# CX9898/BSMR-SDDMM

Hardware: AMD Instinct MI355X
Metric: SDDMM GFLOP/s (higher is better)
Workload: dtype f16

## Files before the change

### bsmr-sddmm_amd/csrc/bsmr_capi.hip

```cpp

#include "bsmr_hip.h"

#include <hip/hip_runtime.h>
#include <hipcub/hipcub.hpp>

#include <algorithm>
#include <chrono>
#include <cmath>
#include <cstdio>
#include <cstdlib>
#include <cstring>
#include <initializer_list>
#include <map>
#include <memory>
#include <mutex>
#include <new>
#include <set>
#include <string>
#include <type_traits>
#include <vector>

#include "dev_array.hpp"
#include "cluster_kernels.hpp"
#include "pack_device.hpp"
// ... 37 lines not shown
    uint32_t H = 0;
    DevArray<uint32_t> groupRows;
    DevArray<uint32_t> blockCols;
    DevArray<uint32_t> blockInfo;
    DevArray<uint32_t> entries;
    DevArray<bsmr::TileItem> items;
    DevArray<uint32_t> itemRowBase;
    uint32_t numItems = 0, entryCap = 0, blocksPerItem = 0;
    uint64_t numBlocks = 0, numTiles = 0, unionColumns = 0, bytes = 0;
};

struct SweepFormatDev {
    uint32_t W = 0, PW = 0, stripBlocks = 0;
    DevArray<uint32_t> panelRows;
    DevArray<bsmr::SweepItem> items;
    DevArray<uint32_t> starts;
    DevArray<uint32_t> rowStart;
    DevArray<uint32_t> words;
    uint32_t numItems = 0, numGroups = 0, numStrips = 0, maxStepEntries = 0, maxItemWords = 0;
    uint64_t bytes = 0;
    bool usable = false;
};

struct GemmFormatDev {
    uint32_t PM = 0, NB = 0;
    DevArray<uint32_t> panelRows;
    DevArray<uint32_t> colOf;
    DevArray<bsmr::GemmItem> items;
    DevArray<uint32_t> rowStart;
    DevArray<uint32_t> lists;
    DevArray<uint32_t> words;
    uint32_t numItems = 0, numGroups = 0, numStrips = 0;
    uint64_t numTiles = 0, bytes = 0;
    bool fullGrid = false, usable = false;
};

struct bsmr_plan {
    int device = 0;
    uint32_t M = 0, N = 0, nnz = 0, numPanels = 0;

    DenseFormat fmt[2];
    uint64_t numDenseEntries = 0;

    DevArray<uint32_t> panelRows;
    DevArray<uint32_t> entryCol;
    DevArray<uint32_t> entryDst;
    DevArray<uint8_t> entryRow;
    DevArray<SparseItem> sparseItems;
    uint64_t numSparseEntries = 0;
    uint32_t numSparseItems = 0;

    uint64_t indexBytes = 0;

    DevArray<uint16_t> A16;
    DevArray<uint16_t> B16;
    uint32_t reservedK = 0;

    int sparseLpe = 0;
    bool sparseLowp = true;
    bool convertInKernel = false;
    DevArray<uint32_t> entryRowId;
    bool sparseFree = false;
    uint64_t foldedEntries = 0;
    uint64_t promotedEntries = 0;
    uint64_t evictedEntries = 0;
    bool groupedDeferred = false;
    bsmr::PackOptions groupedOpt;
// ... 1179 lines not shown
    std::stable_sort(order.begin(), order.end());
    const uint32_t pick = order[std::min<size_t>((size_t)rank, order.size() - 1)].second;
    PM = kGemmShapes[pick][0];
    NB = kGemmShapes[pick][1];
}

int ensureGemm(bsmr_plan* p, uint32_t K) {
    uint32_t PM, NB;
    gemmShape(p, K, PM, NB);
    p->gemmNow = -1;
    if (!gemmShapeBuilt(PM, NB, gemmFp32(p, K))) return BSMR_OK;
    for (size_t i = 0; i < p->gemms.size(); ++i)
        if (p->gemms[i].PM == PM && p->gemms[i].NB == NB) {
            if (p->gemms[i].usable) p->gemmNow = (int)i;
            return BSMR_OK;
        }
    try {
        GemmFormatDev w;
        w.PM = PM;
        w.NB = NB;
        bsmr::GemmFormatHost host;
        int st = bsmr::packGemm(p->hostDense, PM, NB, host, p->opt.gemm_balance_columns != 0);
        if (st == BSMR_ERR_BAD_PLAN || st == BSMR_ERR_INVALID_ARG) {
            p->gemms.push_back(std::move(w));
            return BSMR_OK;
        }
        if (st != BSMR_OK) return st;
        uint64_t bytes = 0;
        w.numItems = (uint32_t)host.items.size();
        w.numGroups = host.numGroups;
        w.numStrips = host.numStrips;
        w.numTiles = host.numTiles;
        w.fullGrid = host.fullGrid;
        st = upload(w.panelRows, host.panelRows, bytes);
        if (st == BSMR_OK) st = upload(w.colOf, host.colOf, bytes);
        if (st == BSMR_OK) st = upload(w.items, host.items, bytes);
        if (st == BSMR_OK) st = upload(w.rowStart, host.rowStart, bytes);
        if (st == BSMR_OK) st = upload(w.lists, host.lists, bytes);
        if (st == BSMR_OK) st = upload(w.words, host.words, bytes);
        if (st != BSMR_OK) return st;
        w.bytes = bytes;
        w.usable = w.numItems != 0;
        p->gemms.push_back(std::move(w));
        p->indexBytes += bytes;
        if (p->gemms.back().usable) p->gemmNow = (int)p->gemms.size() - 1;
        return BSMR_OK;
    } catch (const std::bad_alloc&) {
        return BSMR_ERR_OOM;
    }
}

template <int KT, int PM, int NB, int MODE, bool SRC32>
int launchGemmT(const GemmFormatDev& w, const bsmr_plan* p, const void* A, const void* B, float* P, const Queue& s) {
    const uint64_t K = (SRC32 ? 32u : 64u) * KT, esz = SRC32 ? 4 : 2;
    const uint32_t aBytes = (uint32_t)((uint64_t)p->M * K * esz), bBytes = (uint32_t)((uint64_t)p->N * K * esz);
    const dim3 grid(w.numItems, s.batch.count), block(bsmr::kGemmWaves * bsmr::kWave);
    if constexpr (SRC32) {
        auto kernel = bsmr::denseGemmCvt<KT, PM, NB, MODE>;
        const size_t lds = bsmr::gemmCvtLdsBytes(PM, NB);
        if (int st = raiseDynamicLds(reinterpret_cast<const void*>(kernel), lds, p->device)) return st;
        hipLaunchKernelGGL(kernel, grid, block, lds, s, static_cast<const float*>(A), static_cast<const float*>(B), aBytes, bBytes, w.panelRows,
                           w.colOf, w.items, w.rowStart, w.lists, w.words, P, p->N, w.numGroups, w.numStrips, w.fullGrid ? 1u : 0u, s.batch);
    } else {
        auto kernel = bsmr::denseGemm<KT, PM, NB, MODE, false>;
        const size_t lds = bsmr::gemmLdsBytes(PM, NB);
        if (int st = raiseDynamicLds(reinterpret_cast<const void*>(kernel), lds, p->device)) return st;
        hipLaunchKernelGGL(kernel, grid, block, lds, s, A, B, aBytes, bBytes, w.panelRows, w.colOf, w.items, w.rowStart, w.lists, w.words, P, p->N,
                           w.numGroups, w.numStrips, w.fullGrid ? 1u : 0u, s.batch);
    }
    BSMR_HIP(hipGetLastError());
    return BSMR_OK;
}
template <int KT, int MODE, bool SRC32>
int launchGemmS(const GemmFormatDev& w, const bsmr_plan* p, const void* A, const void* B, float* P, const Queue& s) {
    switch (w.PM * 100 + w.NB) {
    case 1616: return launchGemmT<KT, 16, 16, MODE, SRC32>(w, p, A, B, P, s);
    case 1620: return launchGemmT<KT, 16, 20, MODE, SRC32>(w, p, A, B, P, s);
    case 816: return launchGemmT<KT, 8, 16, MODE, SRC32>(w, p, A, B, P, s);
    case 820: return launchGemmT<KT, 8, 20, MODE, SRC32>(w, p, A, B, P, s);
    case 1612:
        if constexpr (!SRC32) return launchGemmT<KT, 16, 12, MODE, false>(w, p, A, B, P, s);
        return BSMR_ERR_INVALID_ARG;
    default: return BSMR_ERR_INVALID_ARG;
    }
}
template <int MODE>
int launchGemm(const bsmr_plan* p, uint32_t K, const void* A, const void* B, float* P, const Queue& s, bool src32) {
    const GemmFormatDev& w = p->gemms[(size_t)p->gemmNow];
    if (w.numItems == 0) return BSMR_OK;
    if (src32) {
        switch (K) {
        case 64: return launchGemmS<2, MODE, true>(w, p, A, B, P, s);
        case 128: return launchGemmS<4, MODE, true>(w, p, A, B, P, s);
        default: return BSMR_ERR_INVALID_ARG;
        }
    }
    switch (K) {
    case 64: return launchGemmS<1, MODE, false>(w, p, A, B, P, s);
    case 128: return launchGemmS<2, MODE, false>(w, p, A, B, P, s);
    case 256: return launchGemmS<4, MODE, false>(w, p, A, B, P, s);
    case 512: return launchGemmS<8, MODE, false>(w, p, A, B, P, s);
// ... 1945 lines not shown
```

### bsmr-sddmm_amd/csrc/gemm_format.hpp

```cpp
#pragma once

#include <algorithm>
#include <cstdint>
#include <vector>

#include "bsmr_hip.h"
#include "tile_format.hpp"

namespace bsmr {

constexpr uint32_t kGemmWavesM = 2, kGemmWavesN = 4, kGemmWaves = kGemmWavesM * kGemmWavesN;
__host__ __device__ constexpr uint32_t gemmSlabSlot(uint32_t tp, uint32_t r, uint32_t c) { return tp * 256u + (r & 3u) * 64u + (r >> 2) * 16u + c; }
constexpr uint32_t kGemmPassTiles = 16;
constexpr uint32_t kGemmNoEntry = 0xFFFFFFFFu;
constexpr uint32_t kGemmMaxOffset = 8191u;
constexpr uint32_t kGemmSlabStrips = 8;
constexpr uint32_t kGemmWordSlack = 1024;
constexpr uint32_t kGemmMaxRowTiles = 8, kGemmMaxPasses = 3;

struct GemmItem {
    uint32_t group;
    uint32_t firstBlock;
    uint32_t listBase;
    uint32_t pad;
};

__host__ __device__ inline void gemmItemPlace(uint32_t i, uint32_t G, uint32_t S, uint32_t& group, uint32_t& strip) {
    const uint32_t slabs = (S + kGemmSlabStrips - 1u) / kGemmSlabStrips;
    uint32_t slab = i / (kGemmSlabStrips * G);
    if (slab >= slabs) slab = slabs - 1u;
    const uint32_t width = slab + 1u < slabs ? kGemmSlabStrips : S - kGemmSlabStrips * (slabs - 1u);
    const uint32_t rem = i - slab * kGemmSlabStrips * G;
    group = rem / width;
    strip = slab * kGemmSlabStrips + rem % width;
}

struct GemmFormatHost {
    uint32_t PM = 0, NB = 0, numGroups = 0, numStrips = 0, passes = 0;
    bool fullGrid = false;
    std::vector<uint32_t> panelRows;
    std::vector<uint32_t> colOf;
    std::vector<GemmItem> items;
    std::vector<uint32_t> rowStart;
    std::vector<uint32_t> lists;
    std::vector<uint32_t> words;
    uint64_t numTiles = 0;
    uint32_t maxListWords = 0;
    size_t bytes() const {
        return 4 * (panelRows.size() + colOf.size() + rowStart.size() + lists.size() + words.size()) + sizeof(GemmItem) * items.size();
    }
};

inline bool gemmShapeOk(uint32_t PM, uint32_t NB) {
    return (PM == 8 || PM == 16) && (NB == 8 || NB == 12 || NB == 16 || NB == 20);
}

inline int packGemm(const HostDense& hd, uint32_t PM, uint32_t NB, GemmFormatHost& out, bool balanceColumns = true) {
    if (!gemmShapeOk(PM, NB)) return BSMR_ERR_INVALID_ARG;
    const uint32_t P = hd.numPanels, TM = PM * 16;
    const uint32_t G = (P + PM - 1) / PM, NCB = (hd.N + 15) / 16, S = (NCB + NB - 1) / NB;
    const uint32_t m = PM / kGemmWavesM, n = NB / kGemmWavesN, Q = (m * n + kGemmPassTiles - 1) / kGemmPassTiles, L = kGemmWaves * Q;
    out = GemmFormatHost();
    out.PM = PM; out.NB = NB; out.numGroups = G; out.numStrips = S; out.passes = Q;
    if (P == 0 || NCB == 0 || hd.entries() == 0) return BSMR_OK;
    if ((uint64_t)G * S > 0x3FFFFFFFull || hd.entries() > 0xFFFFFFF0ull) return BSMR_ERR_INVALID_ARG;
    if ((uint64_t)hd.nnz * 4u > 0xFFFFFFFCull) return BSMR_ERR_INVALID_ARG;
    out.panelRows.assign((size_t)G * TM, hd.panelRows.empty() ? 0u : hd.panelRows[0]);
    std::vector<uint32_t> rowPos((size_t)P * 16);
    if (balanceColumns) {
        std::vector<uint32_t> weight((size_t)P * 16, 0), order((size_t)P * 16);
        for (uint32_t p = 0; p < P; ++p)
            for (uint64_t e = hd.offsets[p]; e < hd.offsets[p + 1]; ++e) ++weight[(size_t)p * 16 + hd.row[e]];
        for (uint32_t i = 0; i < P * 16; ++i) order[i] = i;
        std::stable_sort(order.begin(), order.end(), [&](uint32_t a, uint32_t b) { return weight[a] > weight[b]; });
        const uint32_t bins = 2 * G, half = TM / 2;
        uint32_t share[kGemmMaxRowTiles][kGemmMaxPasses] = {};
        for (uint32_t tm = 0; tm < m; ++tm)
            for (uint32_t tn = 0; tn < n; ++tn) ++share[tm][(tm * n + tn) / kGemmPassTiles];
        std::vector<uint64_t> load((size_t)bins * Q, 0);
        std::vector<uint8_t> rowsIn((size_t)bins * m, 0);
        for (uint32_t rank = 0; rank < P * 16; ++rank) {
            const uint32_t round = rank / bins, pos = rank % bins, bin = (round & 1u) ? bins - 1u - pos : pos;
            const uint64_t w = weight[order[rank]];
            uint64_t* ld = &load[(size_t)bin * Q];
// ... 14 lines not shown
    for (uint32_t i = 0; i < P * 16; ++i) out.panelRows[rowPos[i]] = hd.panelRows[i];
    const uint32_t TN = NB * 16;
    std::vector<uint32_t> slotOf(hd.N);
    out.colOf.assign((size_t)S * TN, 0u);
    if (balanceColumns) {
        std::vector<uint32_t> degree(hd.N, 0), hot;
        for (uint64_t e = 0; e < hd.entries(); ++e) ++degree[hd.col[e]];
        uint64_t fullest = 0;
        for (uint32_t st = 0; st < S; ++st) {
            uint64_t sum = 0;
            for (uint32_t c = st * TN; c < std::min<uint64_t>(hd.N, (uint64_t)(st + 1) * TN); ++c) sum += degree[c];
            fullest = std::max(fullest, sum);
        }
        const bool lopsided = fullest * S > 2ull * hd.entries();
        const uint64_t threshold = lopsided ? 2ull * hd.entries() / std::max<uint32_t>(1u, hd.N) + 1ull : ~0ull;
        for (uint32_t c = 0; c < hd.N; ++c)
            if (degree[c] > threshold) hot.push_back(c);
        std::stable_sort(hot.begin(), hot.end(), [&](uint32_t a, uint32_t b) { return degree[a] > degree[b]; });
        std::vector<uint32_t> filled(S, 0);
        for (uint32_t rank = 0; rank < hot.size(); ++rank) {
            const uint32_t round = rank / S, pos = rank % S, strip = (round & 1u) ? S - 1u - pos : pos;
            slotOf[hot[rank]] = strip * TN + filled[strip]++;
        }
        uint32_t strip = 0;
        for (uint32_t c = 0; c < hd.N; ++c) {
            if (degree[c] > threshold) continue;
            while (filled[strip] == TN) ++strip;
            slotOf[c] = strip * TN + filled[strip]++;
        }
    } else {
        for (uint32_t c = 0; c < hd.N; ++c) slotOf[c] = c;
    }
    for (uint32_t c = 0; c < hd.N; ++c) out.colOf[slotOf[c]] = c;
    std::vector<uint32_t> itemOf((size_t)G * S, 0xFFFFFFFFu);
    std::vector<uint8_t> used((size_t)G * S, 0);
    for (uint32_t p = 0; p < P; ++p)
        for (uint64_t e = hd.offsets[p]; e < hd.offsets[p + 1]; ++e)
            used[(size_t)(rowPos[(size_t)p * 16 + hd.row[e]] / TM) * S + slotOf[hd.col[e]] / TN] = 1;
    for (uint32_t i = 0; i < G * S; ++i) {
        uint32_t g, st;
        gemmItemPlace(i, G, S, g, st);
        if (!used[(size_t)g * S + st]) continue;
        itemOf[(size_t)g * S + st] = (uint32_t)out.items.size();
        GemmItem it;
        it.group = g;
        it.firstBlock = st * NB;
        it.listBase = (uint32_t)(out.items.size() * (L + 1));
        it.pad = 0;
        out.items.push_back(it);
    }
    out.fullGrid = out.items.size() == (size_t)G * S;
    const size_t I = out.items.size();
    out.numTiles = (uint64_t)I * PM * NB;
    if (I * (size_t)(L + 1) > 0xFFFFFFFFull || I * (size_t)TM > 0xFFFFFFFFull) return BSMR_ERR_INVALID_ARG;
    out.lists.assign(I * (L + 1), 0);
    out.rowStart.assign(I * TM, 0xFFFFFFFFu);
    auto locate = [&](uint32_t p, uint64_t e, size_t& item, uint32_t& list, uint32_t& slot, uint32_t& rowInWave, uint32_t& rowInTile) {
        const uint32_t place = rowPos[(size_t)p * 16 + hd.row[e]];
        const uint32_t g = place / TM, pj = (place % TM) / 16u;
        const uint32_t slotCol = slotOf[hd.col[e]];
        const uint32_t cb = slotCol >> 4, s = cb / NB, bj = cb % NB;
        const uint32_t wm = pj / m, tm = pj % m, wn = bj / n, tn = bj % n;
        const uint32_t t = tm * n + tn, q = t / kGemmPassTiles, tp = t % kGemmPassTiles;
        const uint32_t r = place & 15u, c = slotCol & 15u;
        item = itemOf[(size_t)g * S + s];
        list = (wm * kGemmWavesN + wn) * Q + q;
// ... 58 lines not shown
```

### bsmr-sddmm_amd/csrc/gemm_kernels.hpp

```cpp
#pragma once

#include <hip/hip_runtime.h>
#include <stdint.h>

#include "gemm_format.hpp"
#include "sddmm_kernels.hpp"

namespace bsmr {

constexpr uint32_t kGemmBK = 64;
constexpr uint32_t kGemmRowBytes = kGemmBK * 2u;
__host__ __device__ constexpr uint32_t gemmSwz16(uint32_t row) { return (row >> 1) & 7u; }
__host__ __device__ constexpr uint32_t gemmSwz32(uint32_t row) { return ((row >> 1) & 1u) | (((row >> 3) & 1u) * 6u); }
constexpr uint32_t gemmStageBytes(int PM, int NB) { return (uint32_t)(PM + NB) * 16u * kGemmRowBytes; }
constexpr uint32_t kGemmSlabBytes = kGemmPassTiles * 1024u;
constexpr uint32_t gemmRingBytes(int PM, int NB) {
    return 2u * gemmStageBytes(PM, NB) > kGemmWaves * kGemmSlabBytes ? 2u * gemmStageBytes(PM, NB) : kGemmWaves * kGemmSlabBytes;
}
constexpr size_t gemmLdsBytes(int PM, int NB) { return gemmRingBytes(PM, NB) + (size_t)PM * 16u * 4u; }

#if defined(BSMR_GEMM_LAB)
#define GEMM_LAB_ARG , uint32_t labSkip, unsigned long long* labStamps
#define GEMM_LAB_SKIP(bit) (labSkip & (1u << (bit)))
#define GEMM_LAB_STAMPS unsigned long long labStamp[8] = {0, 0, 0, 0, 0, 0, 0, 0}
// ... 5 lines not shown
#define GEMM_LAB_ARG
#define GEMM_LAB_SKIP(bit) false
#define GEMM_LAB_STAMPS
#define GEMM_LAB_STAMP(i)
#define GEMM_LAB_STAMPS_OUT
#endif

__device__ __forceinline__ void gemmKeep(const u32x4& x) {
#if defined(__HIP_DEVICE_COMPILE__)
    asm volatile("" ::"v"(x));
#else
    (void)x;
#endif
}

constexpr uint32_t kGemmDumpHigh = 64764u;
__device__ __forceinline__ void gemmDumpTile(const f32x4& a, uint32_t tileAddr, bool high) {
#if defined(__HIP_DEVICE_COMPILE__)
#pragma clang diagnostic push
#pragma clang diagnostic ignored "-Winline-asm"
    if (!high)
        asm volatile("s_mov_b32 m0, %4\n\ts_nop 0\n\tds_write_addtid_b32 %0\n\tds_write_addtid_b32 %1 offset:256\n\t"
                     "ds_write_addtid_b32 %2 offset:512\n\tds_write_addtid_b32 %3 offset:768"
                     ::"v"(a[0]), "v"(a[1]), "v"(a[2]), "v"(a[3]), "s"(tileAddr) : "memory", "m0");
    else
        asm volatile("s_mov_b32 m0, %4\n\ts_nop 0\n\tds_write_addtid_b32 %0 offset:64764\n\tds_write_addtid_b32 %1 offset:65020\n\t"
                     "ds_write_addtid_b32 %2 offset:65276\n\tds_write_addtid_b32 %3 offset:65532"
                     ::"v"(a[0]), "v"(a[1]), "v"(a[2]), "v"(a[3]), "s"(tileAddr - kGemmDumpHigh) : "memory", "m0");
#pragma clang diagnostic pop
#else
    (void)a; (void)tileAddr; (void)high;
#endif
}
__device__ __forceinline__ uint32_t gemmLdsAddress(const void* p) {
    return (uint32_t)(uintptr_t)(__attribute__((address_space(3))) const void*)p;
}

template <uint32_t DMAS>
__device__ __forceinline__ void gemmStagePart(const uint8_t* src, uint32_t srcBytes, uint8_t* dst, uint32_t wave, const uint32_t* voff, uint32_t kOff) {
    const auto rsrc = __builtin_amdgcn_make_buffer_rsrc(const_cast<uint8_t*>(src), 0, srcBytes, 0x00020000);
#pragma unroll
    for (uint32_t j = 0; j < DMAS; ++j)
        __builtin_amdgcn_raw_ptr_buffer_load_lds(rsrc, (__attribute__((address_space(3))) void*)(dst + (wave * DMAS + j) * 1024u), 16, voff[j], kOff, 0, 0);
}
__device__ __forceinline__ void gemmStoreEntry(float* P, bool live, uint32_t index, float val) {
    const auto rsrc = __builtin_amdgcn_make_buffer_rsrc(P, 0, 0xFFFFFFFC, 0x00020000);
    __builtin_amdgcn_raw_buffer_store_b32(__builtin_bit_cast(uint32_t, val), rsrc, live ? index << 2 : 0xFFFFFFFFu, 0, 0);
}
template <uint32_t C>
__device__ __forceinline__ void gemmLoadWords(const uint32_t* __restrict__ words, uint32_t e0, uint32_t lane, uint32_t (&w)[C], bool skip) {
    const uint32_t* __restrict__ base = words + e0;
#pragma unroll
    for (uint32_t u = 0; u < C; ++u) w[u] = skip ? kGemmNoEntry : base[u * kWave + lane];
}
template <uint32_t C, uint32_t HALF>
__device__ __forceinline__ void gemmMaskTrip(const float* slab, const uint32_t* rowTable, float* P, uint32_t e, uint32_t last, uint32_t lane,
                                             const uint32_t (&w)[C], bool skipStores) {
#pragma unroll
    for (uint32_t u = 0; u < C; ++u) {
        const bool live = e + u * kWave + lane < last && w[u] != kGemmNoEntry;
        const float val = slab[w[u] & 4095u];
        const uint32_t dst = rowTable[(w[u] >> 12) & (HALF - 1u)] + (w[u] >> 19);
        if (!skipStores) gemmStoreEntry(P, live, dst, val);
    }
}
template <uint32_t C, uint32_t HALF, uint32_t Q, bool DEEP>
__device__ __forceinline__ void gemmMaskPass(const uint32_t* __restrict__ words, const float* slab, const uint32_t* rowTable, float* P,
                                             const uint32_t (&myList)[Q + 1u], uint32_t q, uint32_t lane, uint32_t (&wAhead)[2][C],
                                             bool skipLoads, bool skipStores) {
    const uint32_t first = myList[q], last = myList[q + 1u];
    uint32_t w[C];
#pragma unroll
    for (uint32_t u = 0; u < C; ++u) w[u] = wAhead[q & 1u][u];
    if (DEEP) {
        if (q + 2u < Q) gemmLoadWords<C>(words, myList[q + 2u], lane, wAhead[q & 1u], skipLoads);
    } else if (q + 1u < Q) {
        gemmLoadWords<C>(words, last, lane, wAhead[(q + 1u) & 1u], skipLoads);
    }
    constexpr uint32_t T = C * kWave;
    const bool more = first + T < last;
    uint32_t over[C];
    if (more) gemmLoadWords<C>(words, first + T, lane, over, skipLoads);
    gemmMaskTrip<C, HALF>(slab, rowTable, P, first, last, lane, w, skipStores);
    if (more) {
        for (uint32_t e = first + T; e < last; e += T) {
            uint32_t ahead[C];
            gemmLoadWords<C>(words, e + T, lane, ahead, skipLoads);
            gemmMaskTrip<C, HALF>(slab, rowTable, P, e, last, lane, over, skipStores);
#pragma unroll
            for (uint32_t u = 0; u < C; ++u) over[u] = ahead[u];
        }
    }
}
template <uint32_t ADMAS, uint32_t BDMAS>
__device__ __forceinline__ void gemmStage(const uint8_t* A, uint32_t aBytes, const uint8_t* B, uint32_t bBytes, uint8_t* stage, uint32_t bAt,
                                          uint32_t wave, const uint32_t* voffA, const uint32_t* voffB, uint32_t kOff) {
    gemmStagePart<BDMAS>(B, bBytes, stage + bAt, wave, voffB, kOff);
    gemmStagePart<ADMAS>(A, aBytes, stage, wave, voffA, kOff);
}
__device__ __forceinline__ uint32_t gemmRowOfLane(const uint32_t* __restrict__ rows8, uint32_t sub) {
    uint32_t id = rows8[0];
#pragma unroll
    for (uint32_t k = 1; k < 8; ++k) id = sub == k ? rows8[k] : id;
    return id;
}

template <int KT, int PM, int NB, int MODE, bool SRC32 = false>
__global__ void __launch_bounds__(kGemmWaves * kWave, 2)
denseGemm(const void* __restrict__ Aop, const void* __restrict__ Bop, uint32_t aBytes, uint32_t bBytes,
          const uint32_t* __restrict__ panelRows, const uint32_t* __restrict__ colOf, const GemmItem* __restrict__ items,
          const uint32_t* __restrict__ rowStart,
          const uint32_t* __restrict__ lists, const uint32_t* __restrict__ words, float* __restrict__ P, uint32_t N,
          uint32_t gridG, uint32_t gridS, uint32_t fullGrid, Batch batch GEMM_LAB_ARG) {
    constexpr uint32_t ESZ = SRC32 ? 4u : 2u, K = (kGemmRowBytes / ESZ) * KT, TM = PM * 16u, TN = NB * 16u;
    constexpr uint32_t KSUB = SRC32 ? 1u : 2u;
    constexpr uint32_t m = PM / kGemmWavesM, n = NB / kGemmWavesN, Q = (m * n + kGemmPassTiles - 1u) / kGemmPassTiles, L = kGemmWaves * Q;
    constexpr uint32_t ADMAS = PM / 4u, BDMAS = NB / 4u;
    static_assert(PM % 4 == 0 && NB % 4 == 0, "a stage is filled in whole 1-KiB pieces per wave");
    constexpr uint32_t stageBytes = gemmStageBytes(PM, NB), bAt = TM * kGemmRowBytes;
    constexpr uint32_t rowTableAt = gemmRingBytes(PM, NB);
    constexpr uint32_t kGemmWordChunk = m * n > 32u ? 4u : 8u;
    constexpr bool kPlainDump = m * n > 32u;

    extern __shared__ __attribute__((aligned(16))) uint8_t lds[];
    const uint32_t itemId = xcdContiguous(blockIdx.x, gridDim.x);
    uint32_t group, firstBlock, listBase;
    if (fullGrid) {
        gemmItemPlace(itemId, gridG, gridS, group, firstBlock);
        firstBlock *= (uint32_t)NB;
        listBase = itemId * (L + 1u);
    } else {
        const GemmItem item = items[itemId];
        group = item.group;
        firstBlock = item.firstBlock;
        listBase = item.listBase;
    }
    const uint32_t wave = __builtin_amdgcn_readfirstlane(threadIdx.x >> 6), lane = threadIdx.x & 63u;
    const uint32_t wm = wave / kGemmWavesN, wn = wave % kGemmWavesN;
    const uint32_t r = lane & 15u, g = lane >> 4;
    GEMM_LAB_STAMPS;
    GEMM_LAB_STAMP(0);

    const uint8_t* Ab = static_cast<const uint8_t*>(Aop) + (size_t)blockIdx.y * batch.strideA * ESZ;
    const uint8_t* Bb = static_cast<const uint8_t*>(Bop) + (size_t)blockIdx.y * batch.strideB * ESZ;
    P += (size_t)blockIdx.y * batch.strideP;

    uint32_t voffA[ADMAS], voffB[BDMAS];
#pragma unroll
    for (uint32_t j = 0; j < BDMAS; ++j) {
        const uint32_t col = 8u * (wave * BDMAS + j) + (lane >> 3);
        const uint32_t id = gemmRowOfLane(colOf + (size_t)firstBlock * 16u + 8u * (wave * BDMAS + j), lane >> 3);
        voffB[j] = id * (K * ESZ) + (((lane & 7u) ^ (SRC32 ? gemmSwz32(col) : gemmSwz16(col))) << 4);
    }
    if (!GEMM_LAB_SKIP(2)) gemmStagePart<BDMAS>(Bb, bBytes, lds + bAt, wave, voffB, 0u);
#pragma unroll
    for (uint32_t j = 0; j < ADMAS; ++j) {
        const uint32_t row = 8u * (wave * ADMAS + j) + (lane >> 3);
        const uint32_t id = gemmRowOfLane(panelRows + (size_t)group * TM + 8u * (wave * ADMAS + j), lane >> 3);
        voffA[j] = id * (K * ESZ) + (((lane & 7u) ^ (SRC32 ? gemmSwz32(row) : gemmSwz16(row))) << 4);
    }
    if (!GEMM_LAB_SKIP(2)) gemmStagePart<ADMAS>(Ab, aBytes, lds, wave, voffA, 0u);
    GEMM_LAB_STAMP(1);
    if (threadIdx.x < TM) reinterpret_cast<uint32_t*>(lds + rowTableAt)[threadIdx.x] = rowStart[(size_t)itemId * TM + threadIdx.x];
    uint32_t myList[Q + 1];
#pragma unroll
    for (uint32_t q = 0; q <= Q; ++q) myList[q] = lists[listBase + wave * Q + q];

    const uint32_t fragOff = r * kGemmRowBytes + ((SRC32 ? (2u * g) ^ gemmSwz32(r) : g ^ gemmSwz16(r)) << 4);
    const uint32_t aRead = wm * (TM / 2u) * kGemmRowBytes + fragOff;
    const uint32_t bRead = bAt + wn * (TN / 4u) * kGemmRowBytes + fragOff;

    f32x4 acc[m][n];
#pragma unroll
    for (uint32_t i = 0; i < m; ++i)
#pragma unroll
        for (uint32_t j = 0; j < n; ++j) acc[i][j] = f32x4{0.f, 0.f, 0.f, 0.f};

    auto loadWords = [&](uint32_t e0, uint32_t (&w)[kGemmWordChunk]) { gemmLoadWords<kGemmWordChunk>(words, e0, lane, w, GEMM_LAB_SKIP(4)); };
    constexpr bool kDeepWords = Q >= 2u && m * n <= 32u;
    uint32_t wAhead[2][kGemmWordChunk];
    constexpr bool kEarlyWords = KT <= 4 && !kPlainDump;
    auto firstWords = [&]() {
        loadWords(myList[0], wAhead[0]);
        if (kDeepWords) loadWords(myList[1], wAhead[1]);
    };
#if !defined(BSMR_GEMM_LATE_WORDS)
    if (kEarlyWords) firstWords();
#endif

    asm volatile("s_waitcnt vmcnt(0)" ::: "memory");
    GEMM_LAB_STAMP(2);
    __builtin_amdgcn_s_barrier();
    GEMM_LAB_STAMP(3);
#if defined(BSMR_GEMM_LATE_WORDS)
    if (kEarlyWords) firstWords();
#endif

#pragma unroll
    for (uint32_t t = 0; t < (uint32_t)KT; ++t) {
        if (t + 1u < (uint32_t)KT && !GEMM_LAB_SKIP(2))
            gemmStage<ADMAS, BDMAS>(Ab, aBytes, Bb, bBytes, lds + ((t + 1u) & 1u) * stageBytes, bAt, wave, voffA, voffB, (t + 1u) * kGemmRowBytes);
        if (!kEarlyWords && t + 1u == (uint32_t)KT) firstWords();
        const uint8_t* base = lds + (t & 1u) * stageBytes;
#pragma unroll
        for (uint32_t s = 0; s < KSUB; ++s) {
            auto fragment = [&](uint32_t at, uint32_t tile, uint32_t tag) -> u32x4 {
                if (GEMM_LAB_SKIP(1)) return u32x4{lane, t, tile, s + tag};
                const uint8_t* src = base + ((at + tile * 16u * kGemmRowBytes) ^ (s << 6));
                if constexpr (SRC32) {
                    const f32x4 lo = *reinterpret_cast<const f32x4*>(src);
                    const f32x4 hi = *reinterpret_cast<const f32x4*>(reinterpret_cast<const uint8_t*>(reinterpret_cast<uintptr_t>(src) ^ 16u));
                    return packLowp<MODE>(lo, hi);
                } else {
                    return *reinterpret_cast<const u32x4*>(src);
                }
            };
            u32x4 bf[n];
#pragma unroll
            for (uint32_t j = 0; j < n; ++j) bf[j] = fragment(bRead, j, 0u);
#pragma unroll
            for (uint32_t i = 0; i < m; ++i) {
                const u32x4 af = fragment(aRead, i, 2u);
                if (!GEMM_LAB_SKIP(0)) {
// ... 31 lines not shown
                for (uint32_t tp = 0; tp < kGemmPassTiles; ++tp) {
                    const uint32_t tIdx = q * kGemmPassTiles + tp;
                    if (tIdx < m * n) gemmDumpTile(acc[tIdx / n][tIdx % n], slabAddr + tp * 1024u, false);
                }
            } else {
#pragma unroll
                for (uint32_t tp = 0; tp < kGemmPassTiles; ++tp) {
                    const uint32_t tIdx = q * kGemmPassTiles + tp;
                    if (tIdx < m * n) gemmDumpTile(acc[tIdx / n][tIdx % n], slabAddr + tp * 1024u, true);
                }
            }
        }
        if (kPlainDump) __builtin_amdgcn_sched_barrier(0);
        gemmMaskPass<kGemmWordChunk, TM / 2u, Q, kDeepWords>(words, slab, rowTable, P, myList, q, lane, wAhead, GEMM_LAB_SKIP(4), GEMM_LAB_SKIP(5));
        GEMM_LAB_STAMP(5u + q);
    }
    GEMM_LAB_STAMPS_OUT;
}

constexpr uint32_t kGemmHalfRowBytes = 64u;
__host__ __device__ constexpr uint32_t gemmSwzH(uint32_t row) { return (4u - ((row >> 2) & 3u)) & 3u; }
constexpr uint32_t gemmCvtRingBytes(int PM, int NB) {
    const uint32_t used = (uint32_t)(PM + NB) * 16u * (kGemmRowBytes + 2u * kGemmHalfRowBytes);
    return used > kGemmWaves * kGemmSlabBytes ? used : kGemmWaves * kGemmSlabBytes;
}
constexpr size_t gemmCvtLdsBytes(int PM, int NB) { return gemmCvtRingBytes(PM, NB) + (size_t)PM * 16u * 4u; }

template <int KT, int PM, int NB, int MODE>
__global__ void __launch_bounds__(kGemmWaves * kWave, 2)
denseGemmCvt(const float* __restrict__ Aop, const float* __restrict__ Bop, uint32_t aBytes, uint32_t bBytes,
             const uint32_t* __restrict__ panelRows, const uint32_t* __restrict__ colOf, const GemmItem* __restrict__ items,
             const uint32_t* __restrict__ rowStart,
             const uint32_t* __restrict__ lists, const uint32_t* __restrict__ words, float* __restrict__ P, uint32_t N,
             uint32_t gridG, uint32_t gridS, uint32_t fullGrid, Batch batch GEMM_LAB_ARG) {
    constexpr uint32_t K = 32u * KT, TM = PM * 16u, TN = NB * 16u, ROWS = TM + TN;
    constexpr uint32_t m = PM / kGemmWavesM, n = NB / kGemmWavesN, Q = (m * n + kGemmPassTiles - 1u) / kGemmPassTiles, L = kGemmWaves * Q;
    constexpr uint32_t ADMAS = PM / 4u, BDMAS = NB / 4u, DMAS = ADMAS + BDMAS;
    constexpr uint32_t fBytes = ROWS * kGemmRowBytes, hBytes = ROWS * kGemmHalfRowBytes, bAtF = TM * kGemmRowBytes, bAtH = TM * kGemmHalfRowBytes;
    constexpr uint32_t hAt = fBytes, rowTableAt = gemmCvtRingBytes(PM, NB);
    constexpr uint32_t kGemmWordChunk = m * n > 32u ? 4u : 8u;

    extern __shared__ __attribute__((aligned(16))) uint8_t lds[];
    const uint32_t itemId = xcdContiguous(blockIdx.x, gridDim.x);
    uint32_t group, firstBlock, listBase;
    if (fullGrid) {
        gemmItemPlace(itemId, gridG, gridS, group, firstBlock);
        firstBlock *= (uint32_t)NB;
        listBase = itemId * (L + 1u);
    } else {
        const GemmItem item = items[itemId];
        group = item.group;
        firstBlock = item.firstBlock;
        listBase = item.listBase;
    }
    const uint32_t wave = __builtin_amdgcn_readfirstlane(threadIdx.x >> 6), lane = threadIdx.x & 63u;
    const uint32_t wm = wave / kGemmWavesN, wn = wave % kGemmWavesN;
    const uint32_t r = lane & 15u, g = lane >> 4;
    GEMM_LAB_STAMPS;
    GEMM_LAB_STAMP(0);
    const uint8_t* Ab = reinterpret_cast<const uint8_t*>(Aop) + (size_t)blockIdx.y * batch.strideA * 4u;
    const uint8_t* Bb = reinterpret_cast<const uint8_t*>(Bop) + (size_t)blockIdx.y * batch.strideB * 4u;
    P += (size_t)blockIdx.y * batch.strideP;

    uint32_t voffA[ADMAS], voffB[BDMAS];
    const uint32_t piece = lane & 7u;
#pragma unroll
    for (uint32_t j = 0; j < BDMAS; ++j)
        voffB[j] = gemmRowOfLane(colOf + (size_t)firstBlock * 16u + 8u * (wave * BDMAS + j), lane >> 3) * (K * 4u) + (piece << 4);
    if (!GEMM_LAB_SKIP(2)) gemmStagePart<BDMAS>(Bb, bBytes, lds + bAtF, wave, voffB, 0u);
#pragma unroll
    for (uint32_t j = 0; j < ADMAS; ++j)
        voffA[j] = gemmRowOfLane(panelRows + (size_t)group * TM + 8u * (wave * ADMAS + j), lane >> 3) * (K * 4u) + (piece << 4);
    if (!GEMM_LAB_SKIP(2)) gemmStagePart<ADMAS>(Ab, aBytes, lds, wave, voffA, 0u);
    GEMM_LAB_STAMP(1);
    if (threadIdx.x < TM) reinterpret_cast<uint32_t*>(lds + rowTableAt)[threadIdx.x] = rowStart[(size_t)itemId * TM + threadIdx.x];
    uint32_t myList[Q + 1];
#pragma unroll
    for (uint32_t q = 0; q <= Q; ++q) myList[q] = lists[listBase + wave * Q + q];

#if defined(BSMR_GEMM_ROUND_SERIAL)
    constexpr uint32_t kRoundBatch = 1u;
#else
    constexpr uint32_t kRoundBatch = 5u;
#endif
    const uint32_t fOfA = wave * ADMAS * 1024u + lane * 16u, fOfB = bAtF + wave * BDMAS * 1024u + lane * 16u;
    auto hOf = [&](uint32_t part, uint32_t firstChunk, uint32_t odd) {
        const uint32_t quarter = (2u * (firstChunk + odd) + (lane >> 5)) & 3u;
        return hAt + part + firstChunk * 512u + (lane >> 3) * kGemmHalfRowBytes + (((piece >> 1) ^ ((4u - quarter) & 3u)) << 4) + ((piece & 1u) << 3);
    };
    const uint32_t hOfA[2] = {hOf(0u, wave * ADMAS, 0u), hOf(0u, wave * ADMAS, 1u)};
    const uint32_t hOfB[2] = {hOf(bAtH, wave * BDMAS, 0u), hOf(bAtH, wave * BDMAS, 1u)};
    auto roundChunks = [&](uint32_t to) {
        if (GEMM_LAB_SKIP(1)) return;
#pragma unroll
        for (uint32_t j0 = 0; j0 < DMAS; j0 += kRoundBatch) {
            f32x4 v[kRoundBatch];
#pragma unroll
            for (uint32_t b = 0; b < kRoundBatch; ++b) {
                const uint32_t j = j0 + b;
                if (j >= DMAS) continue;
                v[b] = j < ADMAS ? *reinterpret_cast<const f32x4*>(lds + fOfA + j * 1024u)
                                 : *reinterpret_cast<const f32x4*>(lds + fOfB + (j - ADMAS) * 1024u);
            }
#pragma unroll
            for (uint32_t b = 0; b < kRoundBatch; ++b) {
                const uint32_t j = j0 + b;
                if (j >= DMAS) continue;
                const uint32_t jj = j < ADMAS ? j : j - ADMAS;
                uint8_t* dst = lds + (j < ADMAS ? hOfA[jj & 1u] : hOfB[jj & 1u]) + jj * 512u + to * hBytes;
                typedef uint32_t u32x2 __attribute__((ext_vector_type(2)));
                u32x2 h;
                if constexpr (MODE == 0) {
                    typedef _Float16 f16x4 __attribute__((ext_vector_type(4)));
                    f16x4 o;
                    o[0] = (_Float16)v[b][0]; o[1] = (_Float16)v[b][1]; o[2] = (_Float16)v[b][2]; o[3] = (_Float16)v[b][3];
                    h = __builtin_bit_cast(u32x2, o);
                } else {
                    typedef __bf16 bf16x4 __attribute__((ext_vector_type(4)));
                    bf16x4 o;
                    o[0] = (__bf16)v[b][0]; o[1] = (__bf16)v[b][1]; o[2] = (__bf16)v[b][2]; o[3] = (__bf16)v[b][3];
                    h = __builtin_bit_cast(u32x2, o);
                }
                *reinterpret_cast<u32x2*>(dst) = h;
            }
        }
    };

    const uint32_t fragOff = r * kGemmHalfRowBytes + ((g ^ gemmSwzH(r)) << 4);
    const uint32_t aRead = wm * (TM / 2u) * kGemmHalfRowBytes + fragOff;
    const uint32_t bRead = bAtH + wn * (TN / 4u) * kGemmHalfRowBytes + fragOff;

    f32x4 acc[m][n];
#pragma unroll
    for (uint32_t i = 0; i < m; ++i)
#pragma unroll
        for (uint32_t j = 0; j < n; ++j) acc[i][j] = f32x4{0.f, 0.f, 0.f, 0.f};
    auto loadWords = [&](uint32_t e0, uint32_t (&w)[kGemmWordChunk]) { gemmLoadWords<kGemmWordChunk>(words, e0, lane, w, GEMM_LAB_SKIP(4)); };
    constexpr bool kDeepWords = Q >= 2u && m * n <= 32u;
    uint32_t wAhead[2][kGemmWordChunk];
    constexpr bool kEarlyWords = KT <= 4;
    auto firstWords = [&]() {
        loadWords(myList[0], wAhead[0]);
        if (kDeepWords) loadWords(myList[1], wAhead[1]);
    };
#if !defined(BSMR_GEMM_LATE_WORDS)
    if (kEarlyWords) firstWords();
#endif

    asm volatile("s_waitcnt vmcnt(0)" ::: "memory");
    GEMM_LAB_STAMP(2);
    roundChunks(0u);
    asm volatile("s_waitcnt lgkmcnt(0)" ::: "memory");
    if (KT > 1 && !GEMM_LAB_SKIP(2)) gemmStage<ADMAS, BDMAS>(Ab, aBytes, Bb, bBytes, lds, bAtF, wave, voffA, voffB, kGemmRowBytes);
    __builtin_amdgcn_s_barrier();
    GEMM_LAB_STAMP(3);
#if defined(BSMR_GEMM_LATE_WORDS)
    if (kEarlyWords) firstWords();
#endif

#pragma unroll
    for (uint32_t t = 0; t < (uint32_t)KT; ++t) {
        if (!kEarlyWords && t + 1u == (uint32_t)KT) firstWords();
        const uint8_t* base = lds + hAt + (t & 1u) * hBytes;
        u32x4 bf[n];
#pragma unroll
        for (uint32_t j = 0; j < n; ++j)
            bf[j] = GEMM_LAB_SKIP(6) ? u32x4{lane, t, j, 0u} : *reinterpret_cast<const u32x4*>(base + bRead + j * 16u * kGemmHalfRowBytes);
#pragma unroll
        for (uint32_t i = 0; i < m; ++i) {
            const u32x4 af = GEMM_LAB_SKIP(6) ? u32x4{lane, t, i, 2u} : *reinterpret_cast<const u32x4*>(base + aRead + i * 16u * kGemmHalfRowBytes);
            if (!GEMM_LAB_SKIP(0)) {
#pragma unroll
                for (uint32_t j = 0; j < n; ++j) acc[i][j] = mfma16<MODE>(af, bf[j], acc[i][j]);
            } else {
                gemmKeep(af);
#pragma unroll
                for (uint32_t j = 0; j < n; ++j) gemmKeep(bf[j]);
            }
        }
        if (t + 1u < (uint32_t)KT) {
            asm volatile("s_waitcnt vmcnt(0)" ::: "memory");
            roundChunks((t + 1u) & 1u);
            asm volatile("s_waitcnt lgkmcnt(0)" ::: "memory");
            if (t + 2u < (uint32_t)KT && !GEMM_LAB_SKIP(2))
                gemmStage<ADMAS, BDMAS>(Ab, aBytes, Bb, bBytes, lds, bAtF, wave, voffA, voffB, (t + 2u) * kGemmRowBytes);
        } else {
            asm volatile("s_waitcnt lgkmcnt(0)" ::: "memory");
        }
        __builtin_amdgcn_s_barrier();
    }

    GEMM_LAB_STAMP(4);
    float* slab = reinterpret_cast<float*>(lds) + wave * (kGemmPassTiles * 256u);
    const uint32_t slabAddr = __builtin_amdgcn_readfirstlane(gemmLdsAddress(slab));
    const uint32_t* rowTable = reinterpret_cast<const uint32_t*>(lds + rowTableAt) + wm * (TM / 2u);
#pragma unroll
// ... 24 lines not shown
```

Before: 16300.

## Streamline GEMM prologue: scalar id loads, identity columns, async row table, partial wait

```diff
diff --git a/bsmr-sddmm_amd/csrc/bsmr_capi.hip b/bsmr-sddmm_amd/csrc/bsmr_capi.hip
--- a/bsmr-sddmm_amd/csrc/bsmr_capi.hip
+++ b/bsmr-sddmm_amd/csrc/bsmr_capi.hip
@@ -93,7 +93,7 @@
     DevArray<uint32_t> words;
     uint32_t numItems = 0, numGroups = 0, numStrips = 0;
     uint64_t numTiles = 0, bytes = 0;
-    bool fullGrid = false, usable = false;
+    bool fullGrid = false, colIdentity = false, usable = false;
 };
 
 struct bsmr_plan {
@@ -1339,6 +1339,7 @@
         w.numStrips = host.numStrips;
         w.numTiles = host.numTiles;
         w.fullGrid = host.fullGrid;
+        w.colIdentity = host.colIdentity;
         st = upload(w.panelRows, host.panelRows, bytes);
         if (st == BSMR_OK) st = upload(w.colOf, host.colOf, bytes);
         if (st == BSMR_OK) st = upload(w.items, host.items, bytes);
@@ -1367,13 +1368,13 @@
         const size_t lds = bsmr::gemmCvtLdsBytes(PM, NB);
         if (int st = raiseDynamicLds(reinterpret_cast<const void*>(kernel), lds, p->device)) return st;
         hipLaunchKernelGGL(kernel, grid, block, lds, s, static_cast<const float*>(A), static_cast<const float*>(B), aBytes, bBytes, w.panelRows,
-                           w.colOf, w.items, w.rowStart, w.lists, w.words, P, p->N, w.numGroups, w.numStrips, w.fullGrid ? 1u : 0u, s.batch);
+                           w.colOf, w.items, w.rowStart, w.lists, w.words, P, p->N, w.numGroups, w.numStrips, w.fullGrid ? 1u : 0u, w.colIdentity ? 1u : 0u, s.batch);
     } else {
         auto kernel = bsmr::denseGemm<KT, PM, NB, MODE, false>;
         const size_t lds = bsmr::gemmLdsBytes(PM, NB);
         if (int st = raiseDynamicLds(reinterpret_cast<const void*>(kernel), lds, p->device)) return st;
         hipLaunchKernelGGL(kernel, grid, block, lds, s, A, B, aBytes, bBytes, w.panelRows, w.colOf, w.items, w.rowStart, w.lists, w.words, P, p->N,
-                           w.numGroups, w.numStrips, w.fullGrid ? 1u : 0u, s.batch);
+                           w.numGroups, w.numStrips, w.fullGrid ? 1u : 0u, w.colIdentity ? 1u : 0u, s.batch);
     }
     BSMR_HIP(hipGetLastError());
     return BSMR_OK;
diff --git a/bsmr-sddmm_amd/csrc/gemm_format.hpp b/bsmr-sddmm_amd/csrc/gemm_format.hpp
--- a/bsmr-sddmm_amd/csrc/gemm_format.hpp
+++ b/bsmr-sddmm_amd/csrc/gemm_format.hpp
@@ -38,6 +38,7 @@
 struct GemmFormatHost {
     uint32_t PM = 0, NB = 0, numGroups = 0, numStrips = 0, passes = 0;
     bool fullGrid = false;
+    bool colIdentity = false;
     std::vector<uint32_t> panelRows;
     std::vector<uint32_t> colOf;
     std::vector<GemmItem> items;
@@ -50,6 +51,13 @@
         return 4 * (panelRows.size() + colOf.size() + rowStart.size() + lists.size() + words.size()) + sizeof(GemmItem) * items.size();
     }
 };
+
+inline bool gemmColIdentity(const std::vector<uint32_t>& colOf, uint32_t N) {
+    if (colOf.size() < N) return false;
+    for (uint32_t i = 0; i < N; ++i)
+        if (colOf[i] != i) return false;
+    return true;
+}
 
 inline bool gemmShapeOk(uint32_t PM, uint32_t NB) {
     return (PM == 8 || PM == 16) && (NB == 8 || NB == 12 || NB == 16 || NB == 20);
@@ -130,6 +138,7 @@
         for (uint32_t c = 0; c < hd.N; ++c) slotOf[c] = c;
     }
     for (uint32_t c = 0; c < hd.N; ++c) out.colOf[slotOf[c]] = c;
+    out.colIdentity = gemmColIdentity(out.colOf, hd.N);
     std::vector<uint32_t> itemOf((size_t)G * S, 0xFFFFFFFFu);
     std::vector<uint8_t> used((size_t)G * S, 0);
     for (uint32_t p = 0; p < P; ++p)
diff --git a/bsmr-sddmm_amd/csrc/gemm_kernels.hpp b/bsmr-sddmm_amd/csrc/gemm_kernels.hpp
--- a/bsmr-sddmm_amd/csrc/gemm_kernels.hpp
+++ b/bsmr-sddmm_amd/csrc/gemm_kernels.hpp
@@ -61,6 +61,11 @@
     (void)a; (void)tileAddr; (void)high;
 #endif
 }
+__device__ __forceinline__ void gemmPin(uint32_t& x) {
+#if defined(__HIP_DEVICE_COMPILE__)
+    asm volatile("" : "+v"(x));
+#endif
+}
 __device__ __forceinline__ uint32_t gemmLdsAddress(const void* p) {
     return (uint32_t)(uintptr_t)(__attribute__((address_space(3))) const void*)p;
 }
@@ -127,12 +132,50 @@
     gemmStagePart<BDMAS>(B, bBytes, stage + bAt, wave, voffB, kOff);
     gemmStagePart<ADMAS>(A, aBytes, stage, wave, voffA, kOff);
 }
-__device__ __forceinline__ uint32_t gemmRowOfLane(const uint32_t* __restrict__ rows8, uint32_t sub) {
-    uint32_t id = rows8[0];
-#pragma unroll
-    for (uint32_t k = 1; k < 8; ++k) id = sub == k ? rows8[k] : id;
-    return id;
-}
+typedef uint32_t u32x8 __attribute__((ext_vector_type(8)));
+template <uint32_t DMAS>
+__device__ __forceinline__ void gemmRequestIds(const uint32_t* __restrict__ ids, uint32_t wave, u32x8 (&chunk)[DMAS]) {
+#pragma unroll
+    for (uint32_t j = 0; j < DMAS; ++j) chunk[j] = *(const __attribute__((address_space(4))) u32x8*)(ids + 8u * (wave * DMAS + j));
+}
+template <uint32_t DMAS>
+__device__ __forceinline__ void gemmChunkIds(const u32x8 (&chunk)[DMAS], uint32_t lane, uint32_t (&id)[DMAS]) {
+    const uint32_t sub = lane >> 3;
+#pragma unroll
+    for (uint32_t j = 0; j < DMAS; ++j) {
+        id[j] = chunk[j][0];
+#pragma unroll
+        for (uint32_t k = 1; k < 8; ++k) id[j] = sub == k ? chunk[j][k] : id[j];
+    }
+}
+template <uint32_t DMAS>
+__device__ __forceinline__ void gemmChunkSlots(uint32_t firstSlot, uint32_t N, uint32_t wave, uint32_t lane, uint32_t (&id)[DMAS]) {
+#pragma unroll
+    for (uint32_t j = 0; j < DMAS; ++j) {
+        const uint32_t slot = firstSlot + 8u * (wave * DMAS + j) + (lane >> 3);
+        id[j] = slot < N ? slot : 0u;
+    }
+}
+template <uint32_t TM>
+__device__ __forceinline__ void gemmStageRowTable(const uint32_t* rowStart, uint32_t itemId, uint8_t* table, uint32_t wave, uint32_t lane) {
+    const uint32_t part = wave % (TM / kWave);
+    const auto rsrc = __builtin_amdgcn_make_buffer_rsrc(const_cast<uint32_t*>(rowStart) + (size_t)itemId * TM, 0, TM * 4u, 0x00020000);
+    __builtin_amdgcn_raw_ptr_buffer_load_lds(rsrc, (__attribute__((address_space(3))) void*)(table + part * (kWave * 4u)), 4, lane * 4u, part * (kWave * 4u), 0, 0);
+}
+template <uint32_t YOUNGER>
+__device__ __forceinline__ void gemmWaitFirstStage(bool drain) {
+    if (drain)
+        asm volatile("s_waitcnt vmcnt(0)" ::: "memory");
+    else
+        asm volatile("s_waitcnt vmcnt(%0)" ::"n"(YOUNGER) : "memory");
+}
+
+#if defined(__HIP_DEVICE_COMPILE__)
+#define GEMM_ARGUMENTS_NOW \
+    asm volatile("" ::"s"(Bop), "s"(bBytes), "s"(N), "s"(gridG), "s"(gridS), "s"(fullGrid), "s"(colIdentity), "s"(batch.strideB), "s"(gridDim.x))
+#else
+#define GEMM_ARGUMENTS_NOW
+#endif
 
 template <int KT, int PM, int NB, int MODE, bool SRC32 = false>
 __global__ void __launch_bounds__(kGemmWaves * kWave, 2)
@@ -140,7 +183,7 @@
           const uint32_t* __restrict__ panelRows, const uint32_t* __restrict__ colOf, const GemmItem* __restrict__ items,
           const uint32_t* __restrict__ rowStart,
           const uint32_t* __restrict__ lists, const uint32_t* __restrict__ words, float* __restrict__ P, uint32_t N,
-          uint32_t gridG, uint32_t gridS, uint32_t fullGrid, Batch batch GEMM_LAB_ARG) {
+          uint32_t gridG, uint32_t gridS, uint32_t fullGrid, uint32_t colIdentity, Batch batch GEMM_LAB_ARG) {
     constexpr uint32_t ESZ = SRC32 ? 4u : 2u, K = (kGemmRowBytes / ESZ) * KT, TM = PM * 16u, TN = NB * 16u;
     constexpr uint32_t KSUB = SRC32 ? 1u : 2u;
     constexpr uint32_t m = PM / kGemmWavesM, n = NB / kGemmWavesN, Q = (m * n + kGemmPassTiles - 1u) / kGemmPassTiles, L = kGemmWaves * Q;
@@ -152,6 +195,7 @@
     constexpr bool kPlainDump = m * n > 32u;
 
     extern __shared__ __attribute__((aligned(16))) uint8_t lds[];
+    GEMM_ARGUMENTS_NOW;
     const uint32_t itemId = xcdContiguous(blockIdx.x, gridDim.x);
     uint32_t group, firstBlock, listBase;
     if (fullGrid) {
@@ -164,6 +208,9 @@
         firstBlock = item.firstBlock;
         listBase = item.listBase;
     }
+    group = __builtin_amdgcn_readfirstlane(group);
+    firstBlock = __builtin_amdgcn_readfirstlane(firstBlock);
+    listBase = __builtin_amdgcn_readfirstlane(listBase);
     const uint32_t wave = __builtin_amdgcn_readfirstlane(threadIdx.x >> 6), lane = threadIdx.x & 63u;
     const uint32_t wm = wave / kGemmWavesN, wn = wave % kGemmWavesN;
     const uint32_t r = lane & 15u, g = lane >> 4;
@@ -174,26 +221,37 @@
     const uint8_t* Bb = static_cast<const uint8_t*>(Bop) + (size_t)blockIdx.y * batch.strideB * ESZ;
     P += (size_t)blockIdx.y * batch.strideP;
 
-    uint32_t voffA[ADMAS], voffB[BDMAS];
+    uint32_t voffA[ADMAS], voffB[BDMAS], idA[ADMAS], idB[BDMAS];
+    u32x8 rawA[ADMAS];
+    if (colIdentity) {
+        gemmChunkSlots<BDMAS>(firstBlock * 16u, N, wave, lane, idB);
+    } else {
+        u32x8 rawB[BDMAS];
+        gemmRequestIds<BDMAS>(colOf + (size_t)firstBlock * 16u, wave, rawB);
+        gemmRequestIds<ADMAS>(panelRows + (size_t)group * TM, wave, rawA);
+        gemmChunkIds<BDMAS>(rawB, lane, idB);
+    }
 #pragma unroll
     for (uint32_t j = 0; j < BDMAS; ++j) {
         const uint32_t col = 8u * (wave * BDMAS + j) + (lane >> 3);
-        const uint32_t id = gemmRowOfLane(colOf + (size_t)firstBlock * 16u + 8u * (wave * BDMAS + j), lane >> 3);
-        voffB[j] = id * (K * ESZ) + (((lane & 7u) ^ (SRC32 ? gemmSwz32(col) : gemmSwz16(col))) << 4);
+        voffB[j] = idB[j] * (K * ESZ) + (((lane & 7u) ^ (SRC32 ? gemmSwz32(col) : gemmSwz16(col))) << 4);
     }
     if (!GEMM_LAB_SKIP(2)) gemmStagePart<BDMAS>(Bb, bBytes, lds + bAt, wave, voffB, 0u);
+    __builtin_amdgcn_sched_barrier(0);
+    uint32_t myList[Q + 1];
+#pragma unroll
+    for (uint32_t q = 0; q <= Q; ++q) myList[q] = lists[listBase + wave * Q + q];
+    if (colIdentity) gemmRequestIds<ADMAS>(panelRows + (size_t)group * TM, wave, rawA);
+    gemmChunkIds<ADMAS>(rawA, lane, idA);
 #pragma unroll
     for (uint32_t j = 0; j < ADMAS; ++j) {
         const uint32_t row = 8u * (wave * ADMAS + j) + (lane >> 3);
-        const uint32_t id = gemmRowOfLane(panelRows + (size_t)group * TM + 8u * (wave * ADMAS + j), lane >> 3);
-        voffA[j] = id * (K * ESZ) + (((lane & 7u) ^ (SRC32 ? gemmSwz32(row) : gemmSwz16(row))) << 4);
+        voffA[j] = idA[j] * (K * ESZ) + (((lane & 7u) ^ (SRC32 ? gemmSwz32(row) : gemmSwz16(row))) << 4);
     }
     if (!GEMM_LAB_SKIP(2)) gemmStagePart<ADMAS>(Ab, aBytes, lds, wave, voffA, 0u);
+    gemmStageRowTable<TM>(rowStart, itemId, lds + rowTableAt, wave, lane);
     GEMM_LAB_STAMP(1);
-    if (threadIdx.x < TM) reinterpret_cast<uint32_t*>(lds + rowTableAt)[threadIdx.x] = rowStart[(size_t)itemId * TM + threadIdx.x];
-    uint32_t myList[Q + 1];
-#pragma unroll
-    for (uint32_t q = 0; q <= Q; ++q) myList[q] = lists[listBase + wave * Q + q];
+    __builtin_amdgcn_sched_barrier(0);
 
     const uint32_t fragOff = r * kGemmRowBytes + ((SRC32 ? (2u * g) ^ gemmSwz32(r) : g ^ gemmSwz16(r)) << 4);
     const uint32_t aRead = wm * (TM / 2u) * kGemmRowBytes + fragOff;
@@ -214,10 +272,13 @@
         if (kDeepWords) loadWords(myList[1], wAhead[1]);
     };
 #if !defined(BSMR_GEMM_LATE_WORDS)
+    constexpr uint32_t kWordsInFlight = kEarlyWords ? kGemmWordChunk * (kDeepWords ? 2u : 1u) : 0u;
     if (kEarlyWords) firstWords();
-#endif
-
-    asm volatile("s_waitcnt vmcnt(0)" ::: "memory");
+#else
+    constexpr uint32_t kWordsInFlight = 0u;
+#endif
+
+    gemmWaitFirstStage<kWordsInFlight>(GEMM_LAB_SKIP(4));
     GEMM_LAB_STAMP(2);
     __builtin_amdgcn_s_barrier();
     GEMM_LAB_STAMP(3);
@@ -315,7 +376,7 @@
              const uint32_t* __restrict__ panelRows, const uint32_t* __restrict__ colOf, const GemmItem* __restrict__ items,
              const uint32_t* __restrict__ rowStart,
              const uint32_t* __restrict__ lists, const uint32_t* __restrict__ words, float* __restrict__ P, uint32_t N,
-             uint32_t gridG, uint32_t gridS, uint32_t fullGrid, Batch batch GEMM_LAB_ARG) {
+             uint32_t gridG, uint32_t gridS, uint32_t fullGrid, uint32_t colIdentity, Batch batch GEMM_LAB_ARG) {
     constexpr uint32_t K = 32u * KT, TM = PM * 16u, TN = NB * 16u, ROWS = TM + TN;
     constexpr uint32_t m = PM / kGemmWavesM, n = NB / kGemmWavesN, Q = (m * n + kGemmPassTiles - 1u) / kGemmPassTiles, L = kGemmWaves * Q;
     constexpr uint32_t ADMAS = PM / 4u, BDMAS = NB / 4u, DMAS = ADMAS + BDMAS;
@@ -324,6 +385,7 @@
     constexpr uint32_t kGemmWordChunk = m * n > 32u ? 4u : 8u;
 
     extern __shared__ __attribute__((aligned(16))) uint8_t lds[];
+    GEMM_ARGUMENTS_NOW;
     const uint32_t itemId = xcdContiguous(blockIdx.x, gridDim.x);
     uint32_t group, firstBlock, listBase;
     if (fullGrid) {
@@ -336,6 +398,9 @@
         firstBlock = item.firstBlock;
         listBase = item.listBase;
     }
+    group = __builtin_amdgcn_readfirstlane(group);
+    firstBlock = __builtin_amdgcn_readfirstlane(firstBlock);
+    listBase = __builtin_amdgcn_readfirstlane(listBase);
     const uint32_t wave = __builtin_amdgcn_readfirstlane(threadIdx.x >> 6), lane = threadIdx.x & 63u;
     const uint32_t wm = wave / kGemmWavesN, wn = wave % kGemmWavesN;
     const uint32_t r = lane & 15u, g = lane >> 4;
@@ -345,21 +410,32 @@
     const uint8_t* Bb = reinterpret_cast<const uint8_t*>(Bop) + (size_t)blockIdx.y * batch.strideB * 4u;
     P += (size_t)blockIdx.y * batch.strideP;
 
-    uint32_t voffA[ADMAS], voffB[BDMAS];
+    uint32_t voffA[ADMAS], voffB[BDMAS], idA[ADMAS], idB[BDMAS];
     const uint32_t piece = lane & 7u;
-#pragma unroll
-    for (uint32_t j = 0; j < BDMAS; ++j)
-        voffB[j] = gemmRowOfLane(colOf + (size_t)firstBlock * 16u + 8u * (wave * BDMAS + j), lane >> 3) * (K * 4u) + (piece << 4);
+    u32x8 rawA[ADMAS];
+    if (colIdentity) {
+        gemmChunkSlots<BDMAS>(firstBlock * 16u, N, wave, lane, idB);
+    } else {
+        u32x8 rawB[BDMAS];
+        gemmRequestIds<BDMAS>(colOf + (size_t)firstBlock * 16u, wave, rawB);
+        gemmRequestIds<ADMAS>(panelRows + (size_t)group * TM, wave, rawA);
+        gemmChunkIds<BDMAS>(rawB, lane, idB);
+    }
+#pragma unroll
+    for (uint32_t j = 0; j < BDMAS; ++j) voffB[j] = idB[j] * (K * 4u) + (piece << 4);
     if (!GEMM_LAB_SKIP(2)) gemmStagePart<BDMAS>(Bb, bBytes, lds + bAtF, wave, voffB, 0u);
-#pragma unroll
-    for (uint32_t j = 0; j < ADMAS; ++j)
-        voffA[j] = gemmRowOfLane(panelRows + (size_t)group * TM + 8u * (wave * ADMAS + j), lane >> 3) * (K * 4u) + (piece << 4);
+    __builtin_amdgcn_sched_barrier(0);
+    uint32_t myList[Q + 1];
+#pragma unroll
+    for (uint32_t q = 0; q <= Q; ++q) myList[q] = lists[listBase + wave * Q + q];
+    if (colIdentity) gemmRequestIds<ADMAS>(panelRows + (size_t)group * TM, wave, rawA);
+    gemmChunkIds<ADMAS>(rawA, lane, idA);
+#pragma unroll
+    for (uint32_t j = 0; j < ADMAS; ++j) voffA[j] = idA[j] * (K * 4u) + (piece << 4);
     if (!GEMM_LAB_SKIP(2)) gemmStagePart<ADMAS>(Ab, aBytes, lds, wave, voffA, 0u);
+    gemmStageRowTable<TM>(rowStart, itemId, lds + rowTableAt, wave, lane);
     GEMM_LAB_STAMP(1);
-    if (threadIdx.x < TM) reinterpret_cast<uint32_t*>(lds + rowTableAt)[threadIdx.x] = rowStart[(size_t)itemId * TM + threadIdx.x];
-    uint32_t myList[Q + 1];
-#pragma unroll
-    for (uint32_t q = 0; q <= Q; ++q) myList[q] = lists[listBase + wave * Q + q];
+    __builtin_amdgcn_sched_barrier(0);
 
 #if defined(BSMR_GEMM_ROUND_SERIAL)
     constexpr uint32_t kRoundBatch = 1u;
@@ -410,8 +486,10 @@
     };
 
     const uint32_t fragOff = r * kGemmHalfRowBytes + ((g ^ gemmSwzH(r)) << 4);
-    const uint32_t aRead = wm * (TM / 2u) * kGemmHalfRowBytes + fragOff;
-    const uint32_t bRead = bAtH + wn * (TN / 4u) * kGemmHalfRowBytes + fragOff;
+    uint32_t aRead = hAt + wm * (TM / 2u) * kGemmHalfRowBytes + fragOff;
+    uint32_t bRead = hAt + bAtH + wn * (TN / 4u) * kGemmHalfRowBytes + fragOff;
+    gemmPin(aRead);
+    gemmPin(bRead);
 
     f32x4 acc[m][n];
 #pragma unroll
@@ -427,10 +505,13 @@
         if (kDeepWords) loadWords(myList[1], wAhead[1]);
     };
 #if !defined(BSMR_GEMM_LATE_WORDS)
+    constexpr uint32_t kWordsInFlight = kEarlyWords ? kGemmWordChunk * (kDeepWords ? 2u : 1u) : 0u;
     if (kEarlyWords) firstWords();
-#endif
-
-    asm volatile("s_waitcnt vmcnt(0)" ::: "memory");
+#else
+    constexpr uint32_t kWordsInFlight = 0u;
+#endif
+
+    gemmWaitFirstStage<kWordsInFlight>(GEMM_LAB_SKIP(4));
     GEMM_LAB_STAMP(2);
     roundChunks(0u);
     asm volatile("s_waitcnt lgkmcnt(0)" ::: "memory");
@@ -444,7 +525,7 @@
 #pragma unroll
     for (uint32_t t = 0; t < (uint32_t)KT; ++t) {
         if (!kEarlyWords && t + 1u == (uint32_t)KT) firstWords();
-        const uint8_t* base = lds + hAt + (t & 1u) * hBytes;
+        const uint8_t* base = lds + (t & 1u) * hBytes;
         u32x4 bf[n];
 #pragma unroll
         for (uint32_t j = 0; j < n; ++j)
```

Measured after the change: 16110. 0.988x the previous value.
